# Contingencyy/CPUGPUPathtracing

Hardware: AMD Instinct MI355X
Metric: Mrays/sec @ 1920x1080, 256 spp (dragon glTF stand-in) (higher is better)
Workload: dtype f32

## Files before the change

### cpugpupathtracing_amd/csrc/device/device_scene.h

```cpp
#pragma once
#include <cstdint>
#include <hip/hip_runtime.h>

#include "cpugpupt_abi.h"

namespace cgpt {

static constexpr uint32_t kLeafBit = 0x80000000u;
static constexpr uint32_t kNoHit = 0xFFFFFFFFu;
#ifndef CGPT_TOP_RECORDS_MAX
#define CGPT_TOP_RECORDS_MAX 256
#endif
static constexpr uint32_t kSmallMeshTris = 8;
static constexpr uint32_t kLdsTrisMax = 16;
static constexpr uint32_t kTopRecords = CGPT_TOP_RECORDS_MAX;

struct DevObject {
    uint32_t kind;
    uint32_t mat_index;
    uint32_t root_code;
    uint32_t tri_base;
    uint32_t n_tris;
    float total_area;
    float sphere_radius, sphere_radius_sq;
// ... 59 lines not shown
```

### cpugpupathtracing_amd/csrc/device/shade_device.hpp

```cpp
#pragma once
#include <hip/hip_runtime.h>

#include "device_scene.h"
#include "kernel_variant.h"
#include "rt_device.hpp"

namespace cgpt {
namespace dev {

struct Hit { V3 pos, normal; uint32_t mat; };

__device__ __forceinline__ V3 smooth_normal(V3 p0, V3 p1, V3 p2, V3 n0, V3 n1, V3 n2, V3 P, V3 d)
{
    const V3 e1 = p1 - p0, e2 = p2 - p0, w = P - p0;
    V3 g = cross(e1, e2);
    const float gg = dot(g, g);
    const float u = dot(cross(w, e2), g) / gg;
    const float v = dot(cross(e1, w), g) / gg;
    const V3 m = (1.0f - u - v) * n0 + u * n1 + v * n2;
    const float l2 = dot(m, m);
    if (!(l2 > 1e-12f)) return n0;
    const float len = sqrtf(l2);
    V3 ns = mk(m.x / len, m.y / len, m.z / len);
    if (dot(g, ns) < 0.0f) g = -g;
// ... 223 lines not shown
struct PathState {
    V3 throughput, energy;
    uint32_t rng, depth;
    bool is_specular;
};

enum : uint32_t { kBounceTerminate = 1u, kBounceShadow = 2u, kBounceEnergy = 4u, kBounceBruteDone = 8u };
enum : uint32_t { kBounceChainShift = 4u, kChainReflect = 1u, kChainRefract = 2u, kChainTir = 3u };

__device__ __forceinline__ bool add_light_hit(const DevSettings& st, PathState& ps, V3 emissive, float intensity)
{
    if (!st.nee || ps.depth == 0 || ps.is_specular) { ps.energy = ps.energy + ps.throughput * emissive * intensity; return true; }
    return false;
}

template <bool COUNT, int LOBES = 0, bool RIS = false>
__device__ __forceinline__ uint32_t shade_bounce(const DevScene& sc, const DevSettings& st, Ray& ray, PathState& ps, Ray& shadow,
                                                 V3& pending, Counters& cnt)
{
    constexpr bool ROUGH_SPECULAR = HasRoughSpecular(LOBES), ROUGH_DIELECTRIC = HasRoughDielectric(LOBES);
    if (ps.depth == 0 && st.debug_mode == 2u) {
        ps.energy = ps.energy + bvh_depth_colour(ray);
        return kBounceTerminate | kBounceEnergy;
    }
    if (ray.obj == kNoHit) return kBounceTerminate;

    const Hit hit = get_hit<COUNT, ReadsSmoothNormals(LOBES), HonoursTransforms(LOBES)>(sc, ray, cnt);
    const Mat mat = load_material(sc, hit.mat);
    if (mat.is_light) return add_light_hit(st, ps, mat.emissive, mat.intensity) ? kBounceTerminate | kBounceEnergy : kBounceTerminate;

    uint32_t result = 0;
    const float diffuse_weight = max_std(0.0f, 1.0f - mat.specular - mat.refractivity);
    if (RIS && sc.n_lights > 0 && st.nee && diffuse_weight > 0.001f) {
        const uint32_t M = st.nee;
        float wsum = 0.0f, w_y = 0.0f, dist_y = 0.0f;
        V3 c_y = mk(0.0f), dir_y = mk(0.0f);
        for (uint32_t j = 0; j < M; ++j) {
            const LightSample ls = sample_light(sc, ps.rng, hit.pos);
            const float u = random_float(ps.rng);
            const float NdotL = dot(hit.normal, ls.to_light);
            const float NLdotL = dot(ls.normal, -ls.to_light);
            const V3 c = nee_unshadowed(sc, mat, ps.throughput, ls, NdotL, NLdotL, diffuse_weight);
            const float w = (NdotL > 0.0f && NLdotL > 0.0f) ? c.x + c.y + c.z : 0.0f;
// ... 208 lines not shown
```

### cpugpupathtracing_amd/csrc/device/trace_steps.hpp

```cpp
#pragma once
#include <hip/hip_runtime.h>

#include "device_scene.h"
#include "fast_div.h"
#include "rt_device.hpp"

namespace cgpt {
namespace dev {

static constexpr uint32_t kStartObject = 0x40000000u;
static constexpr uint32_t kIdle = 0x40000001u;
#ifndef CGPT_LDS_STACK_LEVELS
#define CGPT_LDS_STACK_LEVELS 16
#endif
static constexpr uint32_t kLdsStackLevels = CGPT_LDS_STACK_LEVELS;
#ifndef CGPT_TRACE_BLOCK
#define CGPT_TRACE_BLOCK 256
#endif
static constexpr uint32_t kTraceBlock = CGPT_TRACE_BLOCK;
static constexpr uint32_t kRing = 128;
static constexpr uint32_t kLdsObjects = 31;
static constexpr uint32_t kKindEnd = 0xFFFFFFFFu;
static constexpr uint32_t kTopStride = 20;
static constexpr uint32_t kLdsTopMax = 127;
// ... 56 lines not shown
    coarse = chunk_override ? chunk_override * 64u : (per_fetch >= 512u ? 512u : (per_fetch >= 64u ? per_fetch / 64u * 64u : (per_fetch > 16u ? per_fetch : 16u)));
    const uint64_t fb = (uint64_t)n_waves * 64u * fine_rounds / kWorkCounters;
    fine_below = (uint32_t)(fb > 0x7FFFFFFFull ? 0x7FFFFFFFull : (fb ? fb : 1ull));
}

typedef float nt_f4 __attribute__((ext_vector_type(4)));
__device__ __forceinline__ float4 ld_stream(const float4* p)
{
    const nt_f4 v = __builtin_nontemporal_load(reinterpret_cast<const nt_f4*>(p));
    float4 r; r.x = v.x; r.y = v.y; r.z = v.z; r.w = v.w; return r;
}
__device__ __forceinline__ void st_stream(float4* p, float4 v)
{
    nt_f4 x; x.x = v.x; x.y = v.y; x.z = v.z; x.w = v.w;
    __builtin_nontemporal_store(x, reinterpret_cast<nt_f4*>(p));
}
__device__ __forceinline__ uint32_t ld_stream(const uint32_t* p) { return __builtin_nontemporal_load(p); }
__device__ __forceinline__ void st_stream(uint32_t* p, uint32_t v) { __builtin_nontemporal_store(v, p); }

enum PathOrder : uint32_t { kSampleMajor = 0, kTileMajor = 1, kPixelMajor = 2 };
struct PathGrid {
    uint32_t n_pixels;
    uint32_t tiles_x;
    FastDiv div_tiles_x, div_n_pixels;
    uint32_t n_samples;
    FastDiv div_samples;
    uint32_t order;
};
__device__ __forceinline__ void path_split(const PathGrid& g, uint32_t pid, uint32_t& sample, uint32_t& pixel)
{
// ... 62 lines not shown
    const lds_u32* objtab;
    const lds_u32* top_cache;
    const lds_u32* tri_cache;
    uint32_t n_lds_tris;
    uint32_t* deep_block;
    uint32_t deep_stride;
    uint32_t n_top;
    uint32_t first_code;
    bool tab;
};
__host__ __device__ inline size_t trace_lds_bytes(uint32_t top_records)
{
    return ((size_t)kLdsStackLevels * kTraceBlock + (kTraceBlock / 64) * kRing + (kLdsObjects + 1) * 8 + kLdsTrisMax * 12 + (size_t)top_records * kTopStride) * sizeof(uint32_t);
}

__device__ __forceinline__ TravCtx trav_setup(const DevScene& sc, uint32_t* lds_generic, uint32_t top_records, uint32_t* overflow_base, uint32_t grid_threads, uint32_t lds_tris = 1u)
{
    TravCtx c;
    c.sc = &sc;
    lds_u32* const lds = (lds_u32*)lds_generic;
    c.stack = lds + threadIdx.x;
    c.lds_base = lds;
    c.ring = lds + kLdsStackLevels * kTraceBlock + __builtin_amdgcn_readfirstlane(threadIdx.x >> 6) * kRing;
    lds_u32* const objtab = lds + kLdsStackLevels * kTraceBlock + (kTraceBlock / 64u) * kRing;
    c.tab = sc.n_objects <= kLdsObjects;
    if (c.tab) {
        const uint32_t n_words = sc.n_objects * 8u;
        const uint32_t* src = reinterpret_cast<const uint32_t*>(sc.obj_trace);
        for (uint32_t i = threadIdx.x; i < n_words + 8u; i += kTraceBlock) {
            uint32_t v = i < n_words ? src[i] : (i == n_words ? kKindEnd : 0u);
            if ((i & 7u) == 7u) v = (i < n_words && src[i - 7u] == 0u) ? src[i - 6u] : kStartObject;
            objtab[i] = v;
        }
    } else if (threadIdx.x == 0u) objtab[7] = kStartObject;
    lds_u32* const tri_cache = objtab + (kLdsObjects + 1u) * 8u;
    c.n_lds_tris = lds_tris ? min(sc.n_small_tris, kLdsTrisMax) : 0u;
    for (uint32_t i = threadIdx.x; i < c.n_lds_tris * 12u; i += kTraceBlock) {
        const uint32_t w = i % 12u;
        tri_cache[i] = w == 11u ? 0u : reinterpret_cast<const uint32_t*>(sc.tri_leaf)[w >= 8u ? i + 1u : i];
    }
    c.tri_cache = tri_cache;
    lds_u32* const top_cache = tri_cache + kLdsTrisMax * 12u;
    c.n_top = min(top_records, sc.n_top_records);
    for (uint32_t i = threadIdx.x; i < c.n_top * 16u; i += kTraceBlock)
        top_cache[(i >> 4) * kTopStride + (i & 15u)] = reinterpret_cast<const uint32_t*>(sc.node_pairs)[i];
    __syncthreads();
// ... 6 lines not shown
}

struct Trav {
    V3 d;
    RaySlab rs;
    float t;
    uint32_t obj, tri, depth;
    uint32_t cur_obj, code, sp;
    uint32_t fast_levels;
    V3 wo, wd;
};
static constexpr uint32_t kAnyHitBit = 0x80000000u;
__device__ __forceinline__ bool trav_any_hit(const Trav& r) { return (int32_t)r.depth < 0; }
__device__ __forceinline__ uint32_t trav_depth(const Trav& r) { return r.depth & ~kAnyHitBit; }
__device__ __forceinline__ V3 trav_origin(const Trav& r) { return mk(r.rs.oxy.x, r.rs.oxy.y, r.rs.ozi.x); }

template <bool XFORM> __device__ __forceinline__ V3 trav_world_origin(const Trav& r) { return XFORM ? r.wo : trav_origin(r); }
template <bool XFORM> __device__ __forceinline__ V3 trav_world_dir(const Trav& r) { return XFORM ? r.wd : r.d; }

__device__ __forceinline__ void trav_set_ray(Trav& r, V3 o, V3 d)
{
    const V3 inv = mk(1.0f / d.x, 1.0f / d.y, 1.0f / d.z);
    r.d = d;
    r.fast_levels = has_infinite_component(inv) ? 0u : kLdsStackLevels;
    r.rs = make_ray_slab(o, inv);
}
template <bool XFORM = false, bool TREE = false>
__device__ __forceinline__ void trav_start(const TravCtx& c, Trav& r, V3 o, V3 d, float t, uint32_t obj, uint32_t tri, uint32_t depth)
{
    r.t = t; r.obj = obj; r.tri = tri; r.depth = depth;
// ... 233 lines not shown
```

### cpugpupathtracing_amd/csrc/device/wavefront_kernels.hip

```cpp
#include <hip/hip_runtime.h>

#include <algorithm>
#include <cstdint>
#include <cstddef>
#include <cstdlib>
#include <cstring>
#include <new>
#include <type_traits>
#include <vector>

#include "cpugpupt_abi.h"
#include "ctx_internal.h"
#include "device_scene.h"
#include "fast_div.h"
#include "rt_device.hpp"
#include "shade_device.hpp"
#include "shade_items.h"
#include "trace_steps.hpp"
#include "accumulate.hpp"
#include "launch_common.h"

namespace cgpt {

using namespace dev;
// ... 15 lines not shown
    uint32_t* list_ext; uint32_t* list_sh;
    uint32_t* seg_ext; uint32_t* seg_sh;
    uint32_t* seg_count;
    uint32_t* seg_prefix;
    uint32_t n_bands;
    uint32_t band_magic;
    uint32_t* plan;
    uint32_t* stack_overflow;
    uint32_t cap;
    uint32_t n_paths;
    PathGrid g;
    uint32_t n_segs, seg_cap;
    uint32_t shade_chunk;
    uint32_t retire_misses;
    uint32_t rot_trace[2], rot_shade;
    unsigned long long* spec_tab;
    uint32_t spec_keys;
    uint32_t spec_epoch;
    uint32_t probe;
    uint32_t probe_lights;
};

static constexpr uint32_t kChainShift = 10u, kChainMax = 0xFFFFu, kFollowerBit = 0x80000000u, kNoLeader = 0xFFFFFFFFu;
static constexpr uint32_t kSameRayBit = 0x40000000u;

__device__ __forceinline__ uint32_t elect_chain_leader(const WfDev& wf, uint32_t chain, uint32_t pid)
{
    const bool want = chain != 0u;
    uint32_t pixel = 0;
    if (want) { uint32_t sample_unused; path_split(wf.g, pid, sample_unused, pixel); }
    uint32_t src = lane_id();
    for (unsigned long long pend = __builtin_amdgcn_ballot_w64(want); pend != 0ull;) {
        const uint32_t f = (uint32_t)__builtin_ctzll(pend);
        const bool m = want && pixel == __builtin_amdgcn_readlane(pixel, f) && chain == __builtin_amdgcn_readlane(chain, f);
        if (m) src = f;
        pend &= ~__builtin_amdgcn_ballot_w64(m);
// ... 11 lines not shown
            }
            if ((uint32_t)cur == tag) { leader = (uint32_t)(cur >> 32); break; }
        }
    }
    return __shfl(leader, (int)src);
}


template <bool COUNT, bool FIRST, bool XFORM = false, bool TREE = false>
__global__ void __launch_bounds__(kTraceBlock, 1) wf_trace(const DevRenderArgs args, const WfDev wf, uint32_t batch_first, const TraceTune tune)
{
    constexpr bool first_round = FIRST;
    constexpr bool STEP = XFORM || TREE;
    const DevScene& sc = args.scene;
    DevCounters* const counters = args.counters;
    const TravCtx ctx = trav_setup(sc, lds_dyn, tune.top_records, wf.stack_overflow, gridDim.x * kTraceBlock, tune.lds_tris);
    lds_u32* const ring = ctx.ring;

    const uint32_t n_ext = first_round ? wf.g.n_pixels : wf.plan[0];
    const uint32_t n_sh = first_round ? 0u : wf.plan[1];
    const uint32_t blocks_ext = (n_ext + 63u) / 64u, n_blocks = blocks_ext + (n_sh + 63u) / 64u;
    const uint32_t n_waves = gridDim.x * (kTraceBlock / 64u);
    BlockWalk walk = first_block(blockIdx.x * (kTraceBlock / 64u) + __builtin_amdgcn_readfirstlane(threadIdx.x >> 6));
    uint32_t block = block_of(walk);
    const uint32_t rot = wf.rot_trace[first_round ? 1 : 0];
    uint32_t ring_count = 0;

    Trav r;
    r.d = mk(0.0f); r.rs = make_ray_slab(r.d, r.d); r.t = 0.0f;
    r.obj = kNoHit; r.tri = 0; r.depth = 0; r.cur_obj = 0; r.code = kIdle; r.sp = 0; r.fast_levels = kLdsStackLevels;
    if (XFORM) { r.wo = mk(0.0f); r.wd = mk(0.0f); trav_set_ray(r, r.wo, r.wd); }
// ... 8 lines not shown
        asm volatile("" : "+v"(slot));
        if (first_round) {
            float4 c; c.x = __uint_as_float(r.obj); c.y = __uint_as_float(r.tri); c.z = __uint_as_float(trav_depth(r)); c.w = r.t;
            st_stream(&wf.px_hit[slot], c);
        } else if (slot >= wf.cap) {
            if (r.obj == kNoHit) {
                const float4 pe = ld_stream(&wf.C[slot]);
                const uint32_t pid = slot - wf.cap;
                float4 en = ld_stream(&wf.st_en[pid]);
                en.x += pe.x; en.y += pe.y; en.z += pe.z;
                st_stream(&wf.st_en[pid], en);
            }
        } else {
            const bool hit = r.obj != kNoHit;
            if (wf.retire_misses) wf.hit_flag[slot] = hit ? (uint8_t)1 : (uint8_t)0;
            if (!wf.retire_misses || hit) {
                float4 c; c.x = __uint_as_float(r.obj); c.y = __uint_as_float(r.tri); c.z = __uint_as_float(trav_depth(r)); c.w = r.t;
                st_stream(&wf.C[slot], c);
            }
        }
        r.code = kIdle;
    };

    for (;;) {
        const unsigned long long need = __builtin_amdgcn_ballot_w64(r.code == kIdle);
        const uint32_t n_need = (uint32_t)__popcll(need);
        while (ring_count < n_need && block < n_blocks) {
            uint32_t s = 0; bool valid;
            if (block < blocks_ext) {
                const uint32_t i = block * 64u + lane_id();
                valid = i < n_ext;
                if (valid) s = first_round ? i : ld_stream(&wf.list_ext[i]);
            } else {
// ... 80 lines not shown
        }
    }

    const uint32_t per_ray = first_round ? wf.g.n_samples : 1u;
    if (first_round) wave_add_u64(&counters->traced_rays, cnt.rays, per_ray);
    else if (lane_id() == 0u && wave_rays) atomicAdd(&counters->traced_rays, (unsigned long long)wave_rays);
    if (!COUNT && !first_round && lane_id() == 0u && wave_followers) atomicAdd(&counters->chain_followers, (unsigned long long)wave_followers);
    if (!COUNT && !first_round && lane_id() == 0u && wave_unwalked) atomicAdd(&counters->retrace_unwalked, (unsigned long long)wave_unwalked);
    if (COUNT) {
        wave_add_u64(&counters->inner_steps, cnt.inner, per_ray);
        wave_add_u64(&counters->tri_tests, cnt.tris, per_ray);
        wave_add_u64(&counters->bvh_depth_sum, cnt.depth, per_ray);
    }
}

struct ShadeKernArgs { DevRenderArgs args; WfDev wf; uint32_t batch_first; };
static_assert(alignof(DevRenderArgs) == 8 && alignof(WfDev) == 8 && sizeof(DevRenderArgs) % 8 == 0, "ShadeKernArgs mirrors the argument segment: every parameter at its natural alignment");
__device__ __forceinline__ const ShadeKernArgs& shade_kernargs()
{
    const CGPT_UNIFORM ShadeKernArgs* p = (const CGPT_UNIFORM ShadeKernArgs*)__builtin_amdgcn_kernarg_segment_ptr();
    asm volatile("" : "+s"(p));
    return *(const ShadeKernArgs*)p;
}

template <bool COUNT, bool FIRST, bool BRUTE = false, int LOBES = 0, bool RIS = false>
__global__ void __launch_bounds__(256, 1) wf_shade(const DevRenderArgs, const WfDev, uint32_t)
{
    constexpr bool first_round = FIRST;
    constexpr bool kChains = !COUNT && !BRUTE;
    uint32_t n_ext;
    { const WfDev& wf = shade_kernargs().wf; n_ext = first_round ? wf.n_paths : wf.plan[0]; }
    const uint32_t n_blocks = (n_ext + 63u) / 64u;
    const uint32_t n_waves = gridDim.x * 4u;
    const uint32_t wave = blockIdx.x * 4u + __builtin_amdgcn_readfirstlane(threadIdx.x >> 6);
    uint32_t count_ext = 0, count_sh = 0;
    uint32_t cur_band = 0, band_start_ext = 0, band_start_sh = 0;
    Counters cnt = { 0, 0, 0, 0, 0, 0 };
    uint32_t wave_probed = 0;
    uint32_t wave_absorbed = 0;

    BlockWalk walk = first_block(wave);
    const uint32_t chunk = shade_item_blocks(n_blocks, n_waves, shade_kernargs().wf.shade_chunk);
    uint32_t block = wave * chunk;
    auto more = [&]() { return block < n_blocks; };
// ... 31 lines not shown
                queued += (uint32_t)__popcll(m);
                advance();
            }
            if (queued == 0u) break;
            __builtin_amdgcn_wave_barrier();
            const uint32_t take = min(queued, 64u), rest = queued - take;
            active = lane_id() < take;
            if (active) pid = queue[lane_id()];
            const uint32_t moved = queue[64u + lane_id()];
            __builtin_amdgcn_wave_barrier();
            if (lane_id() < rest) queue[lane_id()] = moved;
            __builtin_amdgcn_wave_barrier();
            queued = rest;
        }
        float4 c;
        bool brute_path = false;
        uint32_t sample = 0, px = 0, py = 0;
        if (first_round && active) {
            const ShadeKernArgs& ka = shade_kernargs();
            const DevRenderArgs& args = ka.args;
            uint32_t pixel, local_row;
            path_split(ka.wf.g, pid, sample, pixel);
            active = pixel_of_index(args, ka.wf.g, pixel, px, py, local_row);
            if (active) {
                c = ka.wf.px_hit[pixel];
                if (BRUTE) brute_path = args.settings.render_mode == 1u || (args.settings.render_mode == 0u && px < args.width / 2u);
                if (__float_as_uint(c.x) == kNoHit && args.settings.debug_mode != 2u && !(BRUTE && brute_path)) {
                    if (!pixel_adds_nothing(args, c, px)) {
                        float4 en; en.x = 0.0f; en.y = 0.0f; en.z = 0.0f; en.w = __uint_as_float(0u);
                        st_stream(&ka.wf.st_en[pid], en);
// ... 17 lines not shown
                chain = 1u;
            } else {
                const WfDev& wf = shade_kernargs().wf;
                const float4 a = ld_stream(&wf.A[pid]), b = ld_stream(&wf.B[pid]);
                ray.o = mk(a.x, a.y, a.z); ray.d = mk(b.x, b.y, b.z);
                const float4 tp = ld_stream(&wf.st_tp[pid]);
                ps.throughput = mk(tp.x, tp.y, tp.z); ps.rng = __float_as_uint(tp.w);
                ps.energy = mk(0.0f);
                const uint32_t fl = __float_as_uint(b.w);
                ps.depth = fl & 0xFFu; ps.is_specular = (fl & 0x100u) != 0u;
                if (BRUTE) brute_path = (fl & 0x200u) != 0u;
                if (kChains) chain = (fl >> kChainShift) & kChainMax;
                if (kChains && (fl & kFollowerBit)) {
                    const uint32_t lead = __float_as_uint(a.w);
                    followed = true;
                    if (!wf.retire_misses || wf.hit_flag[lead]) c = ld_stream(&wf.C[lead]);
                    else { c.x = __uint_as_float(kNoHit); c.y = 0.0f; c.z = 0.0f; c.w = 0.0f; }
                } else c = ld_stream(&wf.C[pid]);
            }
            ray.t = c.w; ray.obj = __float_as_uint(c.x); ray.tri = __float_as_uint(c.y); ray.bvh_depth = __float_as_uint(c.z);
            shadow = ray;
            V3 pending = mk(0.0f);

            uint32_t flags = kBounceTerminate;
            if (BRUTE && brute_path) {
                if (is_pixel) {
                    const ShadeKernArgs& ka = shade_kernargs();
                    const DevScene& sc = ka.args.scene;
                    const DevRenderArgs& args = ka.args;
                    const WfDev& wf = ka.wf;
                    const bool done = brute_level<COUNT, LOBES>(sc, args.settings, ray, ps.rng, ps.depth,
                        [&](uint32_t k, const BruteLevel& lv) {
                            float4* rec = wf.brute + ((size_t)k * wf.cap + pid) * 2u;
                            float4 r0, r1;
                            brute_pack(lv, r0, r1);
                            st_stream(&rec[0], r0); st_stream(&rec[1], r1);
                        },
                        [&](uint32_t k) { const float4* rec = wf.brute + ((size_t)k * wf.cap + pid) * 2u; return brute_unpack(ld_stream(&rec[0]), ld_stream(&rec[1])); },
                        ps.energy, cnt);
                    flags = done ? kBounceTerminate | kBounceBruteDone : 0u;
                }
            } else if (is_pixel) {
                const DevRenderArgs& args = shade_kernargs().args;
                flags = shade_bounce<COUNT, LOBES, RIS>(args.scene, args.settings, ray, ps, shadow, pending, cnt);
            }
            if (!COUNT) { absorbed = cnt.unwalked; cnt.unwalked = 0; }
            emit_ext = (flags & kBounceTerminate) == 0u;
            emit_sh = (flags & kBounceShadow) != 0u;
            if (kChains && emit_ext) {
                const uint32_t choice = (flags >> kBounceChainShift) & 3u;
                chain = choice != 0u && chain != 0u && chain <= (kChainMax - 2u) / 3u ? chain * 3u + choice - 1u : 0u;
            }
            bool connect = false;
            bool light_added = false;
            V3 light_energy = mk(0.0f);
            if (!COUNT && shade_kernargs().wf.probe != 0u && !(BRUTE && brute_path)) {
                if (emit_sh) {
                    float t = shadow.t;
                    const uint32_t seen = probe_scene(shade_kernargs().args.scene, shadow.o, shadow.d, t);
// ... 36 lines not shown
                st_stream(&wf.st_tp[pid], tpo);
                float4 na, nb;
                na.x = ray.o.x; na.y = ray.o.y; na.z = ray.o.z; na.w = ray.t;
                nb.x = ray.d.x; nb.y = ray.d.y; nb.z = ray.d.z;
                uint32_t fl = (ps.depth & 0xFFu) | (ps.is_specular ? 0x100u : 0u) | ((BRUTE && brute_path) ? 0x200u : 0u);
                if (((flags >> kBounceChainShift) & 3u) == kChainTir && !(BRUTE && brute_path)) fl |= kSameRayBit;
                if (kChains) {
                    fl |= chain << kChainShift;
                    if (wf.spec_tab) {
                        const uint32_t lead = elect_chain_leader(wf, chain, pid);
                        if (lead != kNoLeader && lead != pid) { na.w = __uint_as_float(lead); fl |= kFollowerBit; }
                    }
                }
                nb.w = __uint_as_float(fl);
                st_stream(&wf.A[pid], na); st_stream(&wf.B[pid], nb);
                if ((first_round || followed) && ray.t != 1e34f) st_stream(&wf.C[pid], c);
                if (first_round && !COUNT && wf.retire_misses && ray.t != 1e34f) wf.hit_flag[pid] = 1;
            }
            if (emit_sh) {
                const uint32_t ss = wf.cap + pid;
                float4 sa, sb, scc;
                sa.x = shadow.o.x; sa.y = shadow.o.y; sa.z = shadow.o.z; sa.w = shadow.t;
                sb.x = shadow.d.x; sb.y = shadow.d.y; sb.z = shadow.d.z; sb.w = 0.0f;
                scc.x = pending.x; scc.y = pending.y; scc.z = pending.z; scc.w = 0.0f;
                st_stream(&wf.A[ss], sa); st_stream(&wf.B[ss], sb); st_stream(&wf.C[ss], scc);
            }
        }
        const unsigned long long m_ext = __builtin_amdgcn_ballot_w64(emit_ext), m_sh = __builtin_amdgcn_ballot_w64(emit_sh);
        if (!COUNT) wave_probed += (uint32_t)__popcll(__builtin_amdgcn_ballot_w64(decided_sh)) + (uint32_t)__popcll(__builtin_amdgcn_ballot_w64(decided_ext));
        if (!COUNT && __builtin_amdgcn_ballot_w64(absorbed != 0u) != 0ull)
            for (uint32_t b = 0; b < 8u; ++b) wave_absorbed += (uint32_t)__popcll(__builtin_amdgcn_ballot_w64((absorbed >> b) & 1u)) << b;
// ... 150 lines not shown
    uint32_t shade_chunk_banded = 32;
    uint32_t shadow_any_hit = 1;
    uint32_t lds_tris = 1;
    uint32_t first_lean = 1;
    uint32_t trace_events = 1;
    uint32_t path_order = 2;
    uint32_t retire_misses = 1;
    uint32_t bands_min_paths = 32u << 20;
    uint32_t bands = 32;
    uint32_t spec_dedupe = 1;
    uint32_t spec_keys = 8;
    uint32_t spec_epochs = 0xFFFF;
    uint32_t probe = 1;
    uint32_t probe_max_objects = 128;
    uint32_t probe_lights = 1;
};

static uint32_t Gcd(uint32_t a, uint32_t b) { while (b) { const uint32_t t = a % b; a = b; b = t; } return a; }
static uint32_t CoprimeRotation(uint32_t n_waves, uint32_t n_tiles)
{
    for (uint32_t rot = 0; rot < n_waves && rot < 4096u; ++rot)
        if (Gcd(n_waves + rot, std::max(1u, n_tiles)) == 1u) return rot;
    return 0u;
}

static decltype(&wf_trace<false, false>) const kTraceKernels[2][2][2] = {
    { { wf_trace<false, false>, wf_trace<false, true> }, { wf_trace<true, false>, wf_trace<true, true> } },
    { { wf_trace<false, false, true>, wf_trace<false, true, true> }, { wf_trace<true, false, true>, wf_trace<true, true, true> } },
};
static decltype(&wf_trace<false, false>) const kTraceTreeKernels[2][2][2] = {
// ... 13 lines not shown
    uint32_t cap = 0, n_pixels = 0, n_segs = 0, seg_cap = 0;
    uint32_t overflow_words = 0;
    uint32_t brute_levels = 0;
    size_t spec = 0;
    bool Holds(const WfSizes& n) const
    {
        return cap >= n.cap && n_pixels >= n.n_pixels && n_segs >= n.n_segs && seg_cap >= n.seg_cap && overflow_words >= n.overflow_words &&
               brute_levels >= n.brute_levels && spec >= n.spec;
    }
};

template <typename F> static void ForEachBuffer(WfDev& d, const WfSizes& s, F&& f)
{
    const size_t slots = 2 * (size_t)s.cap * sizeof(float4), paths = s.cap, segs = (size_t)s.n_segs * s.seg_cap * sizeof(uint32_t);
    const size_t runs = 2 * (size_t)kMaxBands * s.n_segs * sizeof(uint32_t);
    f(d.A, slots); f(d.B, slots); f(d.C, slots);
    f(d.st_tp, paths * sizeof(float4)); f(d.st_en, paths * sizeof(float4)); f(d.hit_flag, paths);
    f(d.px_hit, (size_t)s.n_pixels * sizeof(float4));
    f(d.brute, (size_t)s.brute_levels * paths * 2u * sizeof(float4));
    f(d.list_ext, paths * sizeof(uint32_t)); f(d.list_sh, paths * sizeof(uint32_t));
    f(d.seg_ext, segs); f(d.seg_sh, segs);
    f(d.seg_count, runs); f(d.seg_prefix, runs);
    f(d.plan, (2 + 2 * (size_t)kMaxBands) * sizeof(uint32_t));
    f(d.stack_overflow, (size_t)s.overflow_words * sizeof(uint32_t));
    f(d.spec_tab, s.spec * sizeof(unsigned long long));
}

static size_t PoolBytes(const WfSizes& s)
{
    WfDev d{};
    size_t n = 0;
// ... 64 lines not shown
static const Knob<WfTuning> kKnobs[] = {
    { "pools", &WfTuning::pools, 1, kMaxPools },           { "batch", &WfTuning::batch, 0, 4096 },
    { "max_batch", &WfTuning::max_batch, 1, 4096 },         { "pool_paths_mi", &WfTuning::pool_paths_mi, 1, 1024 },
    { "budget_gib", &WfTuning::budget_gib, 1, 256 },       { "refill", &WfTuning::refill_idle, 1, 64 },
    { "leaf_repeat", &WfTuning::leaf_repeat, 1, 65 },      { "inner_repeat", &WfTuning::inner_repeat, 1, 65 },
    { "obj_repeat", &WfTuning::obj_repeat, 1, 65 },        { "obj_shift", &WfTuning::obj_shift, 0, 6 },
    { "top_records", &WfTuning::top_records, 0, 4096 },     { "trace_blocks", &WfTuning::max_trace_blocks, 1, 64 },
    { "shade_blocks", &WfTuning::max_shade_blocks, 1, 64 },
    { "shade_chunk", &WfTuning::shade_chunk, 1, 256 },     { "shade_chunk_banded", &WfTuning::shade_chunk_banded, 1, 256 },
    { "shadow_any_hit", &WfTuning::shadow_any_hit, 0, 1 },     { "trace_events", &WfTuning::trace_events, 0, 1 },
    { "path_order", &WfTuning::path_order, 0, 2 },         { "retire_misses", &WfTuning::retire_misses, 0, 1 },
    { "lds_tris", &WfTuning::lds_tris, 0, 1 },             { "first_lean", &WfTuning::first_lean, 0, 1 },                     { "bands", &WfTuning::bands, 1, kMaxBands },             { "bands_min_paths", &WfTuning::bands_min_paths, 0, 0x7FFFFFFF },
    { "spec_dedupe", &WfTuning::spec_dedupe, 0, 1 },       { "spec_keys", &WfTuning::spec_keys, 1, 16 },
    { "spec_epochs", &WfTuning::spec_epochs, 1, 0xFFFF },   { "probe", &WfTuning::probe, 0, 1 },
    { "probe_max_objects", &WfTuning::probe_max_objects, 0, 4096 }, { "probe_lights", &WfTuning::probe_lights, 0, 1 },
};

static WfHost* WfGetHost(cgpt_ctx* ctx)
{
    void** slot = CtxWavefrontSlot(ctx);
    if (*slot) return static_cast<WfHost*>(*slot);
    WfHost* fresh = new (std::nothrow) WfHost;
    if (!fresh) { CtxFail(ctx, CGPT_ERR_INVALID, "out of host memory"); return nullptr; }
    LoadKnobsFromEnv(kKnobs, "CGPT_WF_", fresh->tune);
    hipError_t e = hipEventCreateWithFlags(&fresh->begin, hipEventDisableTiming);
    for (uint32_t p = 0; p < kMaxPools && e == hipSuccess; ++p) {
        e = hipStreamCreateWithFlags(&fresh->streams[p], hipStreamNonBlocking);
        if (e == hipSuccess) e = hipEventCreateWithFlags(&fresh->acc_done[p], hipEventDisableTiming);
    }
    if (e != hipSuccess) {
// ... 89 lines not shown
    const dim3 trace_grid_first = tl.grid_first, trace_grid_later = tl.grid_later;
    const bool brute = args_in.settings.render_mode != 2u;
    const uint32_t brute_levels = brute ? (uint32_t)args_in.settings.max_ray_depth + 1u : 0u;
    uint32_t shade_blocks[2][2];
    for (int c = 0; c < 2; ++c)
        for (int b = 0; b < 2; ++b) shade_blocks[c][b] = std::min(h->tune.max_shade_blocks, h->shade_blocks_per_cu[v.ris][v.lobe_level][c][b]);
    const dim3 shade_grid(n_cus * shade_blocks[count][brute]);
    const uint32_t n_segs = n_cus * std::max({ shade_blocks[0][0], shade_blocks[1][0], shade_blocks[0][1], shade_blocks[1][1] }) * 4u;
    const uint32_t min_shade_waves = n_cus * std::min({ shade_blocks[0][0], shade_blocks[1][0], shade_blocks[0][1], shade_blocks[1][1] }) * 4u;

    const uint32_t overflow_words = tl.overflow_words;

    uint32_t shade_chunk = h->tune.shade_chunk;
    const bool chains = h->tune.spec_dedupe && !count && !brute;
    const size_t spec_entries = chains ? (size_t)n_pixels * h->tune.spec_keys : 0u;
    const size_t kBytesPerPath = 160 + 32 * (size_t)brute_levels;
    size_t free_b = 0, total_b = 0;
    LAUNCH_TRY(hipMemGetInfo(&free_b, &total_b));
    const size_t held_bytes = (size_t)h->held_pools * PoolBytes(h->held);
    const size_t budget = std::min<size_t>((size_t)h->tune.budget_gib << 30, (free_b + held_bytes) / 2);
    uint32_t batch = h->tune.batch;
    if (batch == 0) {
        batch = 1;
        while (batch < h->tune.max_batch && (uint64_t)n_pixels * batch * 2u <= (uint64_t)pool_paths) batch *= 2u;
    }
    batch = std::max(1u, std::min({ batch, std::max(1u, args_in.n_samples / 2u), args_in.n_samples, pool_paths / n_pixels }));
    WfSizes need;
    need.n_pixels = n_pixels; need.n_segs = n_segs; need.overflow_words = overflow_words; need.brute_levels = brute_levels; need.spec = spec_entries;
    uint32_t n_pools = 0, n_batches = 0;
    for (int attempt = 0;; ++attempt) {
        for (;;) {
// ... 39 lines not shown
        const uint32_t p = k % n_pools;
        hipStream_t st = h->streams[p];
        const uint32_t bn = std::min(batch, args_in.n_samples - done);
        const uint32_t bfirst = args_in.first_sample + done;
        WfDev wf = h->dev[p];
        wf.cap = h->held.cap; wf.n_paths = n_pixels * bn;
        wf.rot_trace[0] = CoprimeRotation(trace_grid_later.x * (kTraceBlock / 64u), tiles_x * tiles_y);
        wf.rot_trace[1] = CoprimeRotation(trace_grid_first.x * (kTraceBlock / 64u), tiles_x * tiles_y);
        wf.rot_shade = CoprimeRotation(shade_grid.x * 4u, std::max(1u, tiles_x * tiles_y / shade_chunk));
        wf.shade_chunk = shade_chunk;
        wf.g = MakePathGrid(n_pixels, tiles_x, bn, h->tune.path_order); wf.n_segs = h->held.n_segs; wf.seg_cap = h->held.seg_cap;
        wf.n_bands = h->tune.bands > 1u && wf.n_paths >= h->tune.bands_min_paths ? h->tune.bands : 1u;
        if (wf.n_bands > 1u)
            wf.band_magic = (uint32_t)std::min<uint64_t>(0xFFFFFFFFull, (((uint64_t)wf.n_bands << 32) + wf.n_paths - 1u) / wf.n_paths);
        wf.retire_misses = h->tune.retire_misses && args_in.settings.debug_mode == 0u ? 1u : 0u;
        if (!chains) wf.spec_tab = nullptr;
        wf.spec_keys = h->tune.spec_keys;
        wf.probe = h->tune.probe && !count && !xform && !tree && args_in.settings.debug_mode == 0u && args_in.scene.n_objects <= h->tune.probe_max_objects ? 1u : 0u;
        wf.probe_lights = h->tune.probe_lights;
        if (k < n_pools) LAUNCH_TRY(hipMemsetAsync(wf.seg_count, 0, 2 * (size_t)kMaxBands * wf.n_segs * sizeof(uint32_t), st));
        for (uint32_t r = 0; r < rounds; ++r) {
            const bool first = r == 0u;
            if (h->tune.trace_events) LAUNCH_TRY(hipEventRecord(NextEvent(h->trace_ev), st));
            hipLaunchKernelGGL(trace_kernels[xform][count][first], first ? trace_grid_first : trace_grid_later, dim3(kTraceBlock), trace_lds, st, args, wf, bfirst, tt);
            if (h->tune.trace_events) LAUNCH_TRY(hipEventRecord(NextEvent(h->trace_ev), st));
            ++launches;
            if (r + 1u < rounds) {
                if (wf.spec_tab) {
                    if (++h->spec_epoch[p] > h->tune.spec_epochs) {
                        LAUNCH_TRY(hipMemsetAsync(wf.spec_tab, 0, h->held.spec * sizeof(unsigned long long), st));
// ... 65 lines not shown
    }
    for (uint32_t j = 0; j < n_sh; ++j) {
        const uint32_t slot = sh_slot(j);
        A[cap + slot] = F4(sh_o[3 * (size_t)j], sh_o[3 * (size_t)j + 1], sh_o[3 * (size_t)j + 2], sh_tmax ? sh_tmax[j] : 1e34f);
        B[cap + slot] = F4(sh_d[3 * (size_t)j], sh_d[3 * (size_t)j + 1], sh_d[3 * (size_t)j + 2], 0.0f);
        C[cap + slot] = F4(1.0f, 1.0f, 1.0f, 0.0f);
        list_sh[j] = slot;
    }
    const uint32_t plan[2] = { n_ext, n_sh };
    std::vector<float4> en(n_sh);
    std::vector<uint8_t> flag(n_ext);

    DevBuf<float4> dA, dB, dC, d_en;
    DevBuf<uint8_t> d_flag;
    DevBuf<uint32_t> d_list_ext, d_list_sh, d_plan, d_overflow;
    HIP_TRY(ctx, dA.Alloc(2 * (size_t)cap)); HIP_TRY(ctx, dB.Alloc(2 * (size_t)cap)); HIP_TRY(ctx, dC.Alloc(2 * (size_t)cap));
    HIP_TRY(ctx, d_en.Alloc(cap)); HIP_TRY(ctx, d_flag.Alloc(cap));
    HIP_TRY(ctx, d_list_ext.Alloc(cap)); HIP_TRY(ctx, d_list_sh.Alloc(cap));
    HIP_TRY(ctx, d_plan.Alloc(2 + 2 * (size_t)kMaxBands)); HIP_TRY(ctx, d_overflow.Alloc(s.tl.overflow_words));
    hipStream_t st = ctx->stream;
    const size_t slot_bytes = 2 * (size_t)cap * sizeof(float4);
    HIP_TRY(ctx, hipMemcpyAsync(dA.p, A.data(), slot_bytes, hipMemcpyHostToDevice, st));
    HIP_TRY(ctx, hipMemcpyAsync(dB.p, B.data(), slot_bytes, hipMemcpyHostToDevice, st));
    HIP_TRY(ctx, hipMemcpyAsync(dC.p, C.data(), slot_bytes, hipMemcpyHostToDevice, st));
    HIP_TRY(ctx, hipMemsetAsync(d_en.p, 0, (size_t)cap * sizeof(float4), st));
    HIP_TRY(ctx, hipMemsetAsync(d_flag.p, 0, cap, st));
    HIP_TRY(ctx, hipMemcpyAsync(d_list_ext.p, list_ext.data(), (size_t)cap * sizeof(uint32_t), hipMemcpyHostToDevice, st));
    HIP_TRY(ctx, hipMemcpyAsync(d_list_sh.p, list_sh.data(), (size_t)cap * sizeof(uint32_t), hipMemcpyHostToDevice, st));
    HIP_TRY(ctx, hipMemsetAsync(d_plan.p, 0, (2 + 2 * (size_t)kMaxBands) * sizeof(uint32_t), st));
    HIP_TRY(ctx, hipMemcpyAsync(d_plan.p, plan, sizeof(plan), hipMemcpyHostToDevice, st));

// ... 106 lines not shown
```

Measured before the change: 23840.

## Record surface triangle and material at trace time to skip hit reconstruction in shade

During later trace rounds the trace kernel writes a small per-path surface record (global triangle index and material, built from the LDS object table) next to the hit buffer. The shade kernel reads it and, for flat-shaded triangle meshes, takes the stored normal and material directly instead of calling get_hit, avoiding dependent loads through object and triangle data. Miss handling also changes: the hit-flag check on chain followers is replaced by zeroing the tri and depth fields of missed entries. The cost is an extra 8-byte store and load per path, a larger C buffer, and reading WfDev through a raw kernarg pointer.

```diff
diff --git a/cpugpupathtracing_amd/csrc/device/device_scene.h b/cpugpupathtracing_amd/csrc/device/device_scene.h
--- a/cpugpupathtracing_amd/csrc/device/device_scene.h
+++ b/cpugpupathtracing_amd/csrc/device/device_scene.h
@@ -8,6 +8,7 @@
 
 static constexpr uint32_t kLeafBit = 0x80000000u;
 static constexpr uint32_t kNoHit = 0xFFFFFFFFu;
+static constexpr uint32_t kSurfValid = 0x80000000u, kSurfAddTri = 0x40000000u, kSurfNoTri = 0xFFFFFFFFu;
 #ifndef CGPT_TOP_RECORDS_MAX
 #define CGPT_TOP_RECORDS_MAX 256
 #endif
diff --git a/cpugpupathtracing_amd/csrc/device/shade_device.hpp b/cpugpupathtracing_amd/csrc/device/shade_device.hpp
--- a/cpugpupathtracing_amd/csrc/device/shade_device.hpp
+++ b/cpugpupathtracing_amd/csrc/device/shade_device.hpp
@@ -261,19 +261,38 @@
     return false;
 }
 
-template <bool COUNT, int LOBES = 0, bool RIS = false>
+template <bool COUNT, int LOBES = 0, bool RIS = false, bool RECORDED = false>
 __device__ __forceinline__ uint32_t shade_bounce(const DevScene& sc, const DevSettings& st, Ray& ray, PathState& ps, Ray& shadow,
-                                                 V3& pending, Counters& cnt)
+                                                 V3& pending, Counters& cnt, uint32_t surf_tri = 0u, uint32_t surf_mat = 0u)
 {
     constexpr bool ROUGH_SPECULAR = HasRoughSpecular(LOBES), ROUGH_DIELECTRIC = HasRoughDielectric(LOBES);
+    static_assert(!RECORDED || (!COUNT && !ReadsSmoothNormals(LOBES) && !HonoursTransforms(LOBES)), "the record stands for get_hit<false, false, false> only");
     if (ps.depth == 0 && st.debug_mode == 2u) {
         ps.energy = ps.energy + bvh_depth_colour(ray);
         return kBounceTerminate | kBounceEnergy;
     }
     if (ray.obj == kNoHit) return kBounceTerminate;
 
-    const Hit hit = get_hit<COUNT, ReadsSmoothNormals(LOBES), HonoursTransforms(LOBES)>(sc, ray, cnt);
-    const Mat mat = load_material(sc, hit.mat);
+    Hit hit;
+    Mat mat;
+    if constexpr (!RECORDED) {
+        hit = get_hit<COUNT, ReadsSmoothNormals(LOBES), HonoursTransforms(LOBES)>(sc, ray, cnt);
+        mat = load_material(sc, hit.mat);
+    } else {
+        const bool recorded = (surf_mat & kSurfValid) != 0u, flat = recorded && surf_tri != kSurfNoTri;
+        float4 n;
+        if (flat) n = sc.tri_normal[surf_tri];
+        if (recorded) mat = load_material(sc, surf_mat & ~kSurfValid);
+        if (flat) {
+            hit.pos = ray.o + ray.d * ray.t;
+            hit.normal = mk(n.x, n.y, n.z);
+            hit.mat = surf_mat & ~kSurfValid;
+        } else {
+            if (recorded && mat.is_light) return add_light_hit(st, ps, mat.emissive, mat.intensity) ? kBounceTerminate | kBounceEnergy : kBounceTerminate;
+            hit = get_hit<COUNT>(sc, ray, cnt);
+            if (!recorded) mat = load_material(sc, hit.mat);
+        }
+    }
     if (mat.is_light) return add_light_hit(st, ps, mat.emissive, mat.intensity) ? kBounceTerminate | kBounceEnergy : kBounceTerminate;
 
     uint32_t result = 0;
diff --git a/cpugpupathtracing_amd/csrc/device/trace_steps.hpp b/cpugpupathtracing_amd/csrc/device/trace_steps.hpp
--- a/cpugpupathtracing_amd/csrc/device/trace_steps.hpp
+++ b/cpugpupathtracing_amd/csrc/device/trace_steps.hpp
@@ -94,6 +94,17 @@
 {
     nt_f4 x; x.x = v.x; x.y = v.y; x.z = v.z; x.w = v.w;
     __builtin_nontemporal_store(x, reinterpret_cast<nt_f4*>(p));
+}
+typedef uint32_t nt_u2 __attribute__((ext_vector_type(2)));
+__device__ __forceinline__ uint2 ld_stream(const uint2* p)
+{
+    const nt_u2 v = __builtin_nontemporal_load(reinterpret_cast<const nt_u2*>(p));
+    uint2 r; r.x = v.x; r.y = v.y; return r;
+}
+__device__ __forceinline__ void st_stream(uint2* p, uint2 v)
+{
+    nt_u2 x; x.x = v.x; x.y = v.y;
+    __builtin_nontemporal_store(x, reinterpret_cast<nt_u2*>(p));
 }
 __device__ __forceinline__ uint32_t ld_stream(const uint32_t* p) { return __builtin_nontemporal_load(p); }
 __device__ __forceinline__ void st_stream(uint32_t* p, uint32_t v) { __builtin_nontemporal_store(v, p); }
@@ -186,6 +197,7 @@
     return ((size_t)kLdsStackLevels * kTraceBlock + (kTraceBlock / 64) * kRing + (kLdsObjects + 1) * 8 + kLdsTrisMax * 12 + (size_t)top_records * kTopStride) * sizeof(uint32_t);
 }
 
+template <bool SURF = false>
 __device__ __forceinline__ TravCtx trav_setup(const DevScene& sc, uint32_t* lds_generic, uint32_t top_records, uint32_t* overflow_base, uint32_t grid_threads, uint32_t lds_tris = 1u)
 {
     TravCtx c;
@@ -202,6 +214,11 @@
         for (uint32_t i = threadIdx.x; i < n_words + 8u; i += kTraceBlock) {
             uint32_t v = i < n_words ? src[i] : (i == n_words ? kKindEnd : 0u);
             if ((i & 7u) == 7u) v = (i < n_words && src[i - 7u] == 0u) ? src[i - 6u] : kStartObject;
+            if (SURF && i < n_words && ((i & 7u) == 5u || (i & 7u) == 6u) && src[i & ~7u] <= 1u) {
+                const DevObject& o = sc.objects[i >> 3];
+                if ((i & 7u) == 5u) v = o.kind == 1u ? kSurfNoTri : o.tri_base;
+                else v = kSurfValid | o.mat_index | (o.kind == 0u ? kSurfAddTri : 0u);
+            }
             objtab[i] = v;
         }
     } else if (threadIdx.x == 0u) objtab[7] = kStartObject;
@@ -238,6 +255,17 @@
 __device__ __forceinline__ bool trav_any_hit(const Trav& r) { return (int32_t)r.depth < 0; }
 __device__ __forceinline__ uint32_t trav_depth(const Trav& r) { return r.depth & ~kAnyHitBit; }
 __device__ __forceinline__ V3 trav_origin(const Trav& r) { return mk(r.rs.oxy.x, r.rs.oxy.y, r.rs.ozi.x); }
+
+__device__ __forceinline__ uint2 surface_record(const TravCtx& c, const Trav& r)
+{
+    uint2 s; s.x = 0u; s.y = 0u;
+    if (c.tab) {
+        const lds_u32* const e = c.objtab + r.obj * 8u;
+        const uint32_t kind = e[0], base = e[5], m = e[6];
+        if (kind <= 1u) { s.x = base + ((m & kSurfAddTri) ? r.tri : 0u); s.y = m & ~kSurfAddTri; }
+    }
+    return s;
+}
 
 template <bool XFORM> __device__ __forceinline__ V3 trav_world_origin(const Trav& r) { return XFORM ? r.wo : trav_origin(r); }
 template <bool XFORM> __device__ __forceinline__ V3 trav_world_dir(const Trav& r) { return XFORM ? r.wd : r.d; }
diff --git a/cpugpupathtracing_amd/csrc/device/wavefront_kernels.hip b/cpugpupathtracing_amd/csrc/device/wavefront_kernels.hip
--- a/cpugpupathtracing_amd/csrc/device/wavefront_kernels.hip
+++ b/cpugpupathtracing_amd/csrc/device/wavefront_kernels.hip
@@ -53,12 +53,23 @@
     uint32_t shade_chunk;
     uint32_t retire_misses;
     uint32_t rot_trace[2], rot_shade;
+    uint32_t surf_on;
     unsigned long long* spec_tab;
     uint32_t spec_keys;
     uint32_t spec_epoch;
     uint32_t probe;
     uint32_t probe_lights;
 };
+static_assert(offsetof(WfDev, surf_on) + sizeof(uint32_t) == offsetof(WfDev, spec_tab), "surf_on fills the padding in front of spec_tab: no field of WfDev moves");
+
+__device__ __forceinline__ uint2* wf_surf(const WfDev& wf) { return reinterpret_cast<uint2*>(wf.C + 2u * (size_t)wf.cap); }
+
+__device__ __forceinline__ const WfDev& trace_kernarg_wf()
+{
+    const CGPT_UNIFORM char* p = (const CGPT_UNIFORM char*)__builtin_amdgcn_kernarg_segment_ptr();
+    asm volatile("" : "+s"(p));
+    return *(const WfDev*)(p + sizeof(DevRenderArgs));
+}
 
 static constexpr uint32_t kChainShift = 10u, kChainMax = 0xFFFFu, kFollowerBit = 0x80000000u, kNoLeader = 0xFFFFFFFFu;
 static constexpr uint32_t kSameRayBit = 0x40000000u;
@@ -100,7 +111,8 @@
     constexpr bool STEP = XFORM || TREE;
     const DevScene& sc = args.scene;
     DevCounters* const counters = args.counters;
-    const TravCtx ctx = trav_setup(sc, lds_dyn, tune.top_records, wf.stack_overflow, gridDim.x * kTraceBlock, tune.lds_tris);
+    constexpr bool SURF = !COUNT && !STEP && !FIRST;
+    const TravCtx ctx = trav_setup<SURF>(sc, lds_dyn, tune.top_records, wf.stack_overflow, gridDim.x * kTraceBlock, tune.lds_tris);
     lds_u32* const ring = ctx.ring;
 
     const uint32_t n_ext = first_round ? wf.g.n_pixels : wf.plan[0];
@@ -139,9 +151,18 @@
         } else {
             const bool hit = r.obj != kNoHit;
             if (wf.retire_misses) wf.hit_flag[slot] = hit ? (uint8_t)1 : (uint8_t)0;
-            if (!wf.retire_misses || hit) {
+            if constexpr (COUNT) {
+                if (!wf.retire_misses || hit) {
+                    float4 c; c.x = __uint_as_float(r.obj); c.y = __uint_as_float(r.tri); c.z = __uint_as_float(trav_depth(r)); c.w = r.t;
+                    st_stream(&wf.C[slot], c);
+                }
+            } else {
                 float4 c; c.x = __uint_as_float(r.obj); c.y = __uint_as_float(r.tri); c.z = __uint_as_float(trav_depth(r)); c.w = r.t;
+                if (wf.retire_misses && !hit) { c.y = __uint_as_float(0u); c.z = __uint_as_float(0u); }
                 st_stream(&wf.C[slot], c);
+            }
+            if constexpr (SURF) {
+                if (hit) st_stream(&wf_surf(trace_kernarg_wf())[slot], surface_record(ctx, r));
             }
         }
         r.code = kIdle;
@@ -252,6 +273,10 @@
     }
 }
 
+static_assert(std::is_same<decltype(&wf_trace<false, false>), void (*)(DevRenderArgs, WfDev, uint32_t, TraceTune)>::value &&
+              alignof(DevRenderArgs) == 8 && alignof(WfDev) == 8 && sizeof(DevRenderArgs) % 8 == 0,
+              "trace_kernarg_wf() finds wf_trace's second argument behind its first");
+
 struct ShadeKernArgs { DevRenderArgs args; WfDev wf; uint32_t batch_first; };
 static_assert(alignof(DevRenderArgs) == 8 && alignof(WfDev) == 8 && sizeof(DevRenderArgs) % 8 == 0, "ShadeKernArgs mirrors the argument segment: every parameter at its natural alignment");
 __device__ __forceinline__ const ShadeKernArgs& shade_kernargs()
@@ -266,6 +291,7 @@
 {
     constexpr bool first_round = FIRST;
     constexpr bool kChains = !COUNT && !BRUTE;
+    constexpr bool kSurf = !COUNT && !ReadsSmoothNormals(LOBES) && !HonoursTransforms(LOBES);
     uint32_t n_ext;
     { const WfDev& wf = shade_kernargs().wf; n_ext = first_round ? wf.n_paths : wf.plan[0]; }
     const uint32_t n_blocks = (n_ext + 63u) / 64u;
@@ -327,6 +353,7 @@
             queued = rest;
         }
         float4 c;
+        uint2 sr; sr.x = 0u; sr.y = 0u;
         bool brute_path = false;
         uint32_t sample = 0, px = 0, py = 0;
         if (first_round && active) {
@@ -374,9 +401,12 @@
                 if (kChains && (fl & kFollowerBit)) {
                     const uint32_t lead = __float_as_uint(a.w);
                     followed = true;
-                    if (!wf.retire_misses || wf.hit_flag[lead]) c = ld_stream(&wf.C[lead]);
-                    else { c.x = __uint_as_float(kNoHit); c.y = 0.0f; c.z = 0.0f; c.w = 0.0f; }
-                } else c = ld_stream(&wf.C[pid]);
+                    c = ld_stream(&wf.C[lead]);
+                    if (kSurf && wf.surf_on != 0u) sr = ld_stream(&wf_surf(wf)[lead]);
+                } else {
+                    c = ld_stream(&wf.C[pid]);
+                    if (kSurf && wf.surf_on != 0u) sr = ld_stream(&wf_surf(wf)[pid]);
+                }
             }
             ray.t = c.w; ray.obj = __float_as_uint(c.x); ray.tri = __float_as_uint(c.y); ray.bvh_depth = __float_as_uint(c.z);
             shadow = ray;
@@ -402,7 +432,7 @@
                 }
             } else if (is_pixel) {
                 const DevRenderArgs& args = shade_kernargs().args;
-                flags = shade_bounce<COUNT, LOBES, RIS>(args.scene, args.settings, ray, ps, shadow, pending, cnt);
+                flags = shade_bounce<COUNT, LOBES, RIS, kSurf && !FIRST>(args.scene, args.settings, ray, ps, shadow, pending, cnt, sr.x, sr.y);
             }
             if (!COUNT) { absorbed = cnt.unwalked; cnt.unwalked = 0; }
             emit_ext = (flags & kBounceTerminate) == 0u;
@@ -469,7 +499,10 @@
                 }
                 nb.w = __uint_as_float(fl);
                 st_stream(&wf.A[pid], na); st_stream(&wf.B[pid], nb);
-                if ((first_round || followed) && ray.t != 1e34f) st_stream(&wf.C[pid], c);
+                if ((first_round || followed) && ray.t != 1e34f) {
+                    st_stream(&wf.C[pid], c);
+                    if (kSurf && wf.surf_on != 0u) st_stream(&wf_surf(wf)[pid], sr);
+                }
                 if (first_round && !COUNT && wf.retire_misses && ray.t != 1e34f) wf.hit_flag[pid] = 1;
             }
             if (emit_sh) {
@@ -650,6 +683,7 @@
     uint32_t probe = 1;
     uint32_t probe_max_objects = 128;
     uint32_t probe_lights = 1;
+    uint32_t surf_record = 1;
 };
 
 static uint32_t Gcd(uint32_t a, uint32_t b) { while (b) { const uint32_t t = a % b; a = b; b = t; } return a; }
@@ -693,7 +727,7 @@
 {
     const size_t slots = 2 * (size_t)s.cap * sizeof(float4), paths = s.cap, segs = (size_t)s.n_segs * s.seg_cap * sizeof(uint32_t);
     const size_t runs = 2 * (size_t)kMaxBands * s.n_segs * sizeof(uint32_t);
-    f(d.A, slots); f(d.B, slots); f(d.C, slots);
+    f(d.A, slots); f(d.B, slots); f(d.C, slots + paths * sizeof(uint2));
     f(d.st_tp, paths * sizeof(float4)); f(d.st_en, paths * sizeof(float4)); f(d.hit_flag, paths);
     f(d.px_hit, (size_t)s.n_pixels * sizeof(float4));
     f(d.brute, (size_t)s.brute_levels * paths * 2u * sizeof(float4));
@@ -788,6 +822,7 @@
     { "spec_dedupe", &WfTuning::spec_dedupe, 0, 1 },       { "spec_keys", &WfTuning::spec_keys, 1, 16 },
     { "spec_epochs", &WfTuning::spec_epochs, 1, 0xFFFF },   { "probe", &WfTuning::probe, 0, 1 },
     { "probe_max_objects", &WfTuning::probe_max_objects, 0, 4096 }, { "probe_lights", &WfTuning::probe_lights, 0, 1 },
+    { "surf_record", &WfTuning::surf_record, 0, 1 },
 };
 
 static WfHost* WfGetHost(cgpt_ctx* ctx)
@@ -907,7 +942,7 @@
     uint32_t shade_chunk = h->tune.shade_chunk;
     const bool chains = h->tune.spec_dedupe && !count && !brute;
     const size_t spec_entries = chains ? (size_t)n_pixels * h->tune.spec_keys : 0u;
-    const size_t kBytesPerPath = 160 + 32 * (size_t)brute_levels;
+    const size_t kBytesPerPath = 168 + 32 * (size_t)brute_levels;
     size_t free_b = 0, total_b = 0;
     LAUNCH_TRY(hipMemGetInfo(&free_b, &total_b));
     const size_t held_bytes = (size_t)h->held_pools * PoolBytes(h->held);
@@ -977,6 +1012,7 @@
         if (wf.n_bands > 1u)
             wf.band_magic = (uint32_t)std::min<uint64_t>(0xFFFFFFFFull, (((uint64_t)wf.n_bands << 32) + wf.n_paths - 1u) / wf.n_paths);
         wf.retire_misses = h->tune.retire_misses && args_in.settings.debug_mode == 0u ? 1u : 0u;
+        wf.surf_on = h->tune.surf_record && !count && !xform && !tree ? 1u : 0u;
         if (!chains) wf.spec_tab = nullptr;
         wf.spec_keys = h->tune.spec_keys;
         wf.probe = h->tune.probe && !count && !xform && !tree && args_in.settings.debug_mode == 0u && args_in.scene.n_objects <= h->tune.probe_max_objects ? 1u : 0u;
@@ -1072,7 +1108,8 @@
     DevBuf<float4> dA, dB, dC, d_en;
     DevBuf<uint8_t> d_flag;
     DevBuf<uint32_t> d_list_ext, d_list_sh, d_plan, d_overflow;
-    HIP_TRY(ctx, dA.Alloc(2 * (size_t)cap)); HIP_TRY(ctx, dB.Alloc(2 * (size_t)cap)); HIP_TRY(ctx, dC.Alloc(2 * (size_t)cap));
+    HIP_TRY(ctx, dA.Alloc(2 * (size_t)cap)); HIP_TRY(ctx, dB.Alloc(2 * (size_t)cap));
+    HIP_TRY(ctx, dC.Alloc(2 * (size_t)cap + ((size_t)cap + 1u) / 2u));
     HIP_TRY(ctx, d_en.Alloc(cap)); HIP_TRY(ctx, d_flag.Alloc(cap));
     HIP_TRY(ctx, d_list_ext.Alloc(cap)); HIP_TRY(ctx, d_list_sh.Alloc(cap));
     HIP_TRY(ctx, d_plan.Alloc(2 + 2 * (size_t)kMaxBands)); HIP_TRY(ctx, d_overflow.Alloc(s.tl.overflow_words));
```

Result: no change. 23740 (-0.4%).
